# kessel/dune-pnp

Measured on AMD Instinct MI355X. Metric: assembled DOFs/s + BiCGStab iters/s, 3-species PNP on pore.msh-refined, higher is better.
Workload: dtype f64; 1 GPU; config 3: stationary 3-ion PNP, test/pore_pnp/pore.msh refined k=4 x 1 mirrored copies; dofs=2214099, dofs_per_gpu=2214099, mesh_vertices=738033, triangles=1470464, parallelism=mesh partition (RCB) x1, preconditioner=ilu0, colors=4, sell_slots=5176768, blocks=5155025

## Files before the change

### dune-pnp_amd/csrc/assemble.hip

```cpp
#include <cstdlib>

#include <hip/hip_ext.h>

#include "element.h"
#include "kernels.h"

namespace pnp {

namespace {

template <int OP, int KC = 0>
__device__ __forceinline__ void store_block(double *__restrict__ vc, int lane, int s,
                                            const double *Kc) {
  constexpr int NK = OpTraits<OP>::NK;
  static_assert(!KC || OP == OP_PNP, "constant planes: the PNP operator only");
  constexpr int Q0 = KC ? 2 : 0;
#ifdef ASM_STORE_PLAIN
  store_vals<NK, Q0>(vc + size_t(s) * NK * kRows, lane, Kc);
#else
  store_vals_nt<NK, Q0>(vc + size_t(s) * NK * kRows, lane, Kc);
#endif
}

template <int NF>
__device__ __forceinline__ void residual_tail(const AsmArgs &a, int row, unsigned fl,
                                              const double (&R)[NF]) {
  double cv[NF];
#pragma unroll
  for (int f = 0; f < NF; f++) cv[f] = 0.0;
  if (fl & kRowFlagLoad) {
#pragma unroll
    for (int f = 0; f < NF; f++) cv[f] = a.cvec[size_t(row) * NF + f];
  }
#pragma unroll
  for (int f = 0; f < NF; f++) {
    const double rv = R[f] + cv[f];
    a.r[size_t(row) * NF + f] = ((fl >> f) & 1) ? 0.0 : rv;
  }
}

template <int OP, int JAC, int MINW, int FANR>
__global__ __launch_bounds__(256, MINW) void k_assemble(DevLayout L, AsmArgs a) {
  using T = OpTraits<OP>;
  constexpr int NF = T::NF, NK = T::NK;
  const int row = xcd_block(blockIdx.x, gridDim.x, L.xcd_remap) * blockDim.x + threadIdx.x;
  if (row >= L.n_owned) return;
  const int chunk = row / kRows, lane = row % kRows;
  const int off = L.chunk_off[chunk];
  const uint64_t meta = L.rowmeta[row];
  const int len = int(meta & 63);
  const bool closed = (meta >> 6) & 1;
  const unsigned brk = unsigned(meta >> 8);
  const int *__restrict__ cix = L.colidx + off + lane;
  double *__restrict__ vc = a.vals + size_t(off) * NK;

  const double2 pi2 = reinterpret_cast<const double2 *>(L.xy)[row];
  double ui[NF];
#pragma unroll
  for (int f = 0; f < NF; f++) ui[f] = a.x[size_t(row) * NF + f];
  double ai = 0, aq = 0;
  if constexpr (OP == OP_DIFF || OP == OP_DIFF_IE || OP == OP_POISSON) ai = a.aux0[row];
  if constexpr (OP == OP_POISSON) aq = a.aux1[row];
  if constexpr (OP == OP_PB) pb_fifth(ui[0], ai, aq);

  double R[NF], D[NK], P[NK], F[NK];
#pragma unroll
  for (int f = 0; f < NF; f++) R[f] = 0;
#pragma unroll
  for (int v = 0; v < NK; v++) D[v] = P[v] = F[v] = 0;

  auto next_slot = [&](int s) { return (s + 1 < len) ? s + 1 : (closed ? 1 : -1); };
  auto load_nb = [&](int j, double2 &p, double (&u)[NF], double &a0, double &a1) {
// ... 70 lines not shown
      for (int v = 0; v < NK; v++) P[v] = 0;
    }
    pc = pn;
#pragma unroll
    for (int f = 0; f < NF; f++) uc[f] = un[f];
    ac0 = an0;
    ac1 = an1;
    if (tn > 0) {
      pn = pp;
#pragma unroll
      for (int f = 0; f < NF; f++) un[f] = up[f];
      an0 = ap0;
      an1 = ap1;
    }
  }
  if constexpr (JAC) {
    if (closed) {
#pragma unroll
      for (int v = 0; v < NK; v++) F[v] += P[v];
      store_block<OP>(vc, lane, 1, F);
    }
    store_block<OP>(vc, lane, 0, D);
  }
  residual_tail<NF>(a, row, a.rowflag[row], R);
}

#ifndef ASM_SU
#define ASM_SU 4
#endif
template <int OP>
__host__ __device__ constexpr int asm_lds_rec() {
  return 2 + OpTraits<OP>::NF + (OP == OP_DIFF || OP == OP_DIFF_IE || OP == OP_POISSON) +
         (OP == OP_POISSON);
}
template <int OP>
constexpr int asm_kc() {
  return OP == OP_PNP;
}
constexpr int kPipeDw = 11;
template <class P>
__device__ __forceinline__ void lds_dma4(const P *src, uint32_t *dst_wave) {
  __builtin_amdgcn_global_load_lds(
      (const __attribute__((address_space(1))) void *)(src),
      (__attribute__((address_space(3))) void *)(dst_wave), 4, 0, 0);
}
__device__ __forceinline__ int const_ld(const int *p, int i) {
  return ((const __attribute__((address_space(4))) int *)(p))[i];
}
__device__ __forceinline__ int row_block_const(const DevLayout &L, int b, int nwg) {
  return L.blkmap ? const_ld(L.blkmap, xcd_block(b, nwg, 1)) : xcd_block(b, nwg, L.xcd_remap);
}
template <int OP, int JAC, int MINW, int FANR, int SPLIT = FANR, int STAGE = 0, int LDSG = 0,
          int KC = 0, int PIPE = 0>
__global__ __launch_bounds__(256, MINW) void k_assemble_ga(DevLayout L, AsmArgs a) {
  using T = OpTraits<OP>;
  constexpr int NF = T::NF, NK = T::NK, NS = FANR;
  constexpr bool AUX0 = OP == OP_DIFF || OP == OP_DIFF_IE || OP == OP_POISSON;
  constexpr bool AUX1 = OP == OP_POISSON;
  constexpr int RW = asm_lds_rec<OP>();
  static_assert(!PIPE || (JAC && FANR == 9 && !STAGE && !LDSG), "PIPE: the direct Jacobian walk");
  extern __shared__ double srec[];
  __shared__ uint32_t pfb[PIPE ? 4 * kPipeDw * kRows : 1];
  const int ntiles = (L.n_owned + 255) / 256, G = gridDim.x;
  const int wv = PIPE ? __builtin_amdgcn_readfirstlane(int(threadIdx.x) / kRows) : 0;
  const int ln = int(threadIdx.x) % kRows;
  uint32_t *const pw = pfb + (PIPE ? wv * kPipeDw * kRows : 0);
  int tile = blockIdx.x, b0 = -1, b1 = -1, b2 = -1, o0 = 0, o1 = 0, c1 = 0;
  auto tile_blk = [&](int t) { return t < ntiles ? row_block_const(L, t, ntiles) : -1; };
  auto wave_chunk = [&](int b) {
    return (b >= 0 && b * 256 + wv * kRows < L.n_owned) ? b * 4 + wv : -1;
  };
  auto prefetch = [&](int b, int off, int clen) {
    if (wave_chunk(b) < 0) return;
    const int r0 = b * 256 + wv * kRows;
    const int *cix = L.colidx + off + ln;
#pragma unroll
    for (int k = 1; k < NS; k++)
      lds_dma4(cix + (k < clen ? k : 0) * kRows, pw + (k - 1) * kRows);
    const uint32_t *m =
        reinterpret_cast<const uint32_t *>(L.rowmeta + min(r0 + ln, L.n_owned - 1));
    lds_dma4(m, pw + 8 * kRows);
    lds_dma4(m + 1, pw + 9 * kRows);
    lds_dma4(reinterpret_cast<const uint32_t *>(a.rowflag + r0) + (ln >> 2), pw + 10 * kRows);
  };
  if constexpr (PIPE) {
    if (tile >= ntiles) return;
    b0 = tile_blk(tile);
    b1 = tile_blk(tile + G);
    b2 = tile_blk(tile + 2 * G);
    int c0 = 0;
    if (wave_chunk(b0) >= 0) {
      o0 = const_ld(L.chunk_off, wave_chunk(b0));
      c0 = const_ld(L.chunk_len, wave_chunk(b0));
    }
    if (wave_chunk(b1) >= 0) {
      o1 = const_ld(L.chunk_off, wave_chunk(b1));
      c1 = const_ld(L.chunk_len, wave_chunk(b1));
    }
    prefetch(b0, o0, c0);
  }
  int o2 = 0, c2 = 0, b3 = -1;
  const auto advance = [&]() {
    tile += G;
    b0 = b1, o0 = o1;
    b1 = b2, o1 = o2, c1 = c2;
    b2 = b3;
    return b0 >= 0;
  };
  do {
    const int blk = PIPE ? b0 : row_block(L, blockIdx.x, gridDim.x);
    const int row0 = blk * blockDim.x + threadIdx.x;
    const bool live = row0 < L.n_owned;
    if (!PIPE && !LDSG && !live) return;
    const int row = live ? row0 : 0;
    const int chunk = row / kRows, lane = row % kRows;
    int cj[NS];
    uint64_t meta_pf = 0;
    unsigned fl_pf = 0;
    if constexpr (PIPE) {
      asm volatile("s_waitcnt vmcnt(0)" ::: "memory");
#pragma unroll
      for (int k = 1; k < NS; k++) cj[k] = int(pw[(k - 1) * kRows + ln]);
      meta_pf = uint64_t(pw[8 * kRows + ln]) | (uint64_t(pw[9 * kRows + ln]) << 32);
      fl_pf = (pw[10 * kRows + ln] >> (8 * (ln & 3))) & 0xffu;
      asm volatile("s_waitcnt lgkmcnt(0)" ::: "memory");
      prefetch(b1, o1, c1);
      o2 = c2 = 0;
      if (wave_chunk(b2) >= 0) {
        o2 = const_ld(L.chunk_off, wave_chunk(b2));
        c2 = const_ld(L.chunk_len, wave_chunk(b2));
      }
      b3 = tile_blk(tile + 3 * G);
      if (!live) continue;
    }
    const int off = PIPE ? o0 : L.chunk_off[chunk];
    const uint64_t meta = PIPE ? meta_pf : L.rowmeta[row];
    const int len = int(meta & 63);
    const bool closed = (meta >> 6) & 1;
    const unsigned brk = unsigned(meta >> 8);
    double *__restrict__ vc = a.vals + size_t(off) * NK;

    if constexpr (PIPE) {
    } else if constexpr (LDSG) {
      const uint16_t *__restrict__ lix = L.lidx + off + lane;
#pragma unroll
      for (int k = 1; k < NS; k++) {
        const int t = lix[(k < len ? k : 0) * kRows];
        cj[k] = k < len ? t : 0;
      }
    } else {
      const int *__restrict__ cix = L.colidx + off + lane;
#pragma unroll
      for (int k = 1; k < NS; k++) cj[k] = cix[(k < len ? k : 0) * kRows];
    }
    const double2 pi2 = reinterpret_cast<const double2 *>(L.xy)[row];
    double ui[NF];
    load_nf<NF>(a.x, size_t(row), ui);
    double ai = 0, aq = 0;
    if constexpr (AUX0) ai = a.aux0[row];
    if constexpr (AUX1) aq = a.aux1[row];
    if constexpr (OP == OP_PB) pb_fifth(ui[0], ai, aq);
    if constexpr (LDSG) {
      const int u0 = L.uptr[blk], cnt = L.uown[blk];
      constexpr int kSU = ASM_SU;
      int jj[kSU];
#pragma unroll
      for (int u = 0; u < kSU; u++) {
        const int k = int(threadIdx.x) + u * 256;
        jj[u] = k < cnt ? L.ulist[u0 + k] : -1;
      }
      double t[kSU][RW];
#pragma unroll
      for (int u = 0; u < kSU; u++)
        if (jj[u] >= 0) {
          const double2 p = reinterpret_cast<const double2 *>(L.xy)[jj[u]];
          t[u][0] = p.x;
          t[u][1] = p.y;
          double uu[NF];
          load_nf<NF>(a.x, size_t(jj[u]), uu);
#pragma unroll
          for (int f = 0; f < NF; f++) t[u][2 + f] = uu[f];
          if constexpr (AUX0) t[u][2 + NF] = a.aux0[jj[u]];
          if constexpr (AUX1) t[u][3 + NF] = a.aux1[jj[u]];
        }
#pragma unroll
      for (int u = 0; u < kSU; u++)
        if (jj[u] >= 0)
#pragma unroll
          for (int w = 0; w < RW; w++) srec[size_t(int(threadIdx.x) + u * 256) * RW + w] = t[u][w];
      for (int k = int(threadIdx.x) + kSU * 256; k < cnt; k += blockDim.x) {
        const int j = L.ulist[u0 + k];
        const double2 p = reinterpret_cast<const double2 *>(L.xy)[j];
        double u[NF];
        load_nf<NF>(a.x, size_t(j), u);
        double *r = srec + size_t(k) * RW;
        r[0] = p.x;
        r[1] = p.y;
#pragma unroll
        for (int f = 0; f < NF; f++) r[2 + f] = u[f];
        if constexpr (AUX0) r[2 + NF] = a.aux0[j];
        if constexpr (AUX1) r[3 + NF] = a.aux1[j];
      }
      __syncthreads();
      if (!live) return;
    }
    double2 pn[NS];
    double un[NS][NF], a0[NS], a1[NS];
    auto gather = [&](int k) {
      if constexpr (LDSG) {
        const double *r = srec + size_t(cj[k]) * RW;
        pn[k] = make_double2(r[0], r[1]);
#pragma unroll
        for (int f = 0; f < NF; f++) un[k][f] = r[2 + f];
// ... 67 lines not shown
#pragma unroll
              for (int v = 0; v < NK; v++) F[v] = P[v];
            } else {
              put(s, P);
            }
#pragma unroll
            for (int v = 0; v < NK; v++) P[v] = Ct[v];
          }
        } else if constexpr (JAC) {
          put(s, P);
#pragma unroll
          for (int v = 0; v < NK; v++) P[v] = 0;
        }
      }
    }
    if constexpr (JAC) {
      if (closed) {
#pragma unroll
        for (int v = 0; v < NK; v++) F[v] += P[v];
        store_block<OP, KC>(vc, lane, 1, F);
      }
      store_block<OP, KC>(vc, lane, 0, D);
    }
    residual_tail<NF>(a, row, PIPE ? fl_pf : unsigned(a.rowflag[row]), R);
  } while (PIPE && advance());
}

template <int OP>
__global__ __launch_bounds__(256) void k_mass_apply(DevLayout L, double tau, double pi, int cyl,
                                                    const double *__restrict__ xo,
                                                    double *__restrict__ cvec) {
  constexpr int NF = OpTraits<OP>::NF;
  const int row = blockIdx.x * blockDim.x + threadIdx.x;
  if (row >= L.n_owned) return;
  const int chunk = row / kRows, lane = row % kRows;
  const int off = L.chunk_off[chunk];
  const uint64_t meta = L.rowmeta[row];
  const int len = int(meta & 63);
  const bool closed = (meta >> 6) & 1;
  const int *cix = L.colidx + off + lane;
  const double2 pi2 = reinterpret_cast<const double2 *>(L.xy)[row];
  double acc = 0;
  for (int s = 1; s < len; ++s) {
    const int t = (s + 1 < len) ? s + 1 : (closed ? 1 : -1);
    if (t < 0 || ((meta >> (8 + s)) & 1)) continue;
    const int b = cix[s * kRows], c = cix[t * kRows];
    const double2 pb2 = reinterpret_cast<const double2 *>(L.xy)[b];
// ... 74 lines not shown
    static const int resident = [&] {
      int dev = 0, cus = 0, per_cu = 0;
      if (hipGetDevice(&dev) != hipSuccess ||
          hipDeviceGetAttribute(&cus, hipDeviceAttributeMultiprocessorCount, dev) != hipSuccess ||
          hipOccupancyMaxActiveBlocksPerMultiprocessor(&per_cu, kern, 256, 0) != hipSuccess)
        return 0;
      return per_cu * cus;
    }();
    const int ntiles = (L.n_owned + 255) / 256;
    int g = resident >= 8 ? resident / 8 * 8 : 8;
    if (g > ntiles) g = ntiles;
    if (cap > 0 && g > cap) g = cap;
    hipExtLaunchKernelGGL(kern, dim3(g), dim3(256), 0, s, t0, t1, 0, L, a);
    return 1;
  } else {
    return 0;
  }
}

hipError_t launch_assemble(const DevLayout &L, const AsmArgs &a, hipStream_t s, hipEvent_t t0,
                           hipEvent_t t1, int *pipelined) {
  if (pipelined) *pipelined = 0;
  if (L.n_owned == 0) return hipSuccess;
  dim3 grid((L.n_owned + 255) / 256), block(256);
  static const int waves = [] {
    const char *e = getenv("PNP_ASM_WAVES");
    return (e && atoi(e) == 4) ? 4 : 3;
  }();
  static const bool fanr_ok = [] {
    const char *e = getenv("PNP_ASM_FANR");
    return !(e && atoi(e) == 0);
  }();
  static const int ga = [] {
    const char *e = getenv("PNP_ASM_GA");
    return e ? atoi(e) : 4;
  }();
  const int fanr = !fanr_ok ? 0 : (L.max_slots <= 9 ? 9 : (L.max_slots <= 12 ? 12 : 0));
  static const int lds_env = [] {
    const char *e = getenv("PNP_ASM_LDS");
    return e ? (atoi(e) == 1 ? 1 : 0) : -1;
  }();
  static const bool cold_hint = [] {
    const char *e = getenv("PNP_ASM_COLD_HINT");
    return !(e && e[0] == '0');
  }();
  const auto lds_walk = [&](int nk) {
// ... 92 lines not shown
```

### dune-pnp_amd/csrc/ctx.cc

```cpp
#include "ctx.h"

static thread_local std::string g_err;
std::mutex g_groups_m;
std::map<std::string, std::shared_ptr<LocalGroup>> g_groups;

void pnp_ctx::asm_wrote(bool kc, bool full) {
  if (kc) {
    asm_reused++;
  } else {
    asm_full++;
    vals_const_valid = full;
  }
}

pnp_ctx::~pnp_ctx() {
  graphs_clear();
  for (auto &v : ev_pending)
    for (auto &pr : v) {
      hipEventDestroy(pr.first);
      hipEventDestroy(pr.second);
    }
  for (auto e : ev_pool) hipEventDestroy(e);
  if (hS) hipHostFree(hS);
  if (h_send) hipHostFree(h_send);
// ... 1655 lines not shown
  view->bseg = mb->m.bseg.data();
  view->bseg_group = mb->m.bgroup.data();
  return PNP_OK;
}

extern "C" void pnp_mesh_free(pnp_mesh_buf *m) { delete m; }

extern "C" const char *pnp_last_error(const pnp_ctx *ctx) {
  return ctx ? ctx->err.c_str() : g_err.c_str();
}

extern "C" int pnp_rccl_unique_id(void *out128) {
  if (!out128) return PNP_E_ARG;
  ncclUniqueId id;
  if (ncclGetUniqueId(&id) != ncclSuccess) {
    g_err = "ncclGetUniqueId failed";
    return PNP_E_RCCL;
  }
  static_assert(sizeof(ncclUniqueId) == 128, "ncclUniqueId size");
  std::memcpy(out128, &id, 128);
  return PNP_OK;
}

static void params_from(const pnp_params *pp, pnp::Params &P) {
  P.l_b = pp->l_b;
  P.c0 = pp->c0;
  P.tau = pp->tau;
  P.pi = pp->pi;
  P.cylindrical = pp->cylindrical;
  P.surf.resize(pp->n_surfaces);
  for (int i = 0; i < pp->n_surfaces; i++) {
    const pnp_surface &s = pp->surfaces[i];
    pnp::Surface &d = P.surf[i];
    d.cb = s.coulomb_btype;
    d.cflux = s.coulomb_flux;
    d.cpot = s.coulomb_potential;
    d.pb = s.plus_btype;
    d.pflux = s.plus_flux;
    d.pconc = s.plus_concentration;
    d.mb = s.minus_btype;
    d.mflux = s.minus_flux;
    d.mconc = s.minus_concentration;
  }
}

#define CK(expr, what)                                 \
// ... 292 lines not shown
        c->h_posrowU[pos] = rowU(pos);
      }
      c->h_lsx_ptr = lp;
      c->h_lsx_list = ll;
      c->h_usx_ptr = up2;
      c->h_usx_list = ul;
      c->ilu_flow[0].built = c->ilu_flow[1].built = false;
    }
  }
  {
    std::vector<int> ro(L.n_owned + 1, 0), rcol;
    rcol.reserve(size_t(L.nblocks));
    for (int i = 0; i < L.n_owned; i++) {
      const int ch = i / pnp::kRows, ln = i % pnp::kRows, len = pnp::meta_len(L.rowmeta[i]);
      for (int sl = 0; sl < len; sl++)
        rcol.push_back(L.colidx[size_t(L.chunk_off[ch]) + 64 * size_t(sl) + ln]);
      ro[i + 1] = ro[i] + len;
    }
    if ((rc = up(c->d_rowoff, ro, "rowoff")) || (rc = up(c->d_rowcol, rcol, "rowcol"))) {
      g_err = c->err;
      return rc;
    }
  }
  {
    const char *e = getenv("PNP_BLKMAP");
    if (!(e && atoi(e) == 0) && L.n_owned > 0) {
      int nblk = (L.n_owned + 255) / 256;
      std::vector<double> key(nblk);
      for (int b = 0; b < nblk; b++) {
        int r = 256 * b, cc = L.rowcolor[r];
        double lo = L.color_ptr[cc], hi = L.color_ptr[cc + 1];
        key[b] = (r - lo) / std::max(1.0, hi - lo);
      }
      std::vector<int> order(nblk);
      for (int b = 0; b < nblk; b++) order[b] = b;
      std::stable_sort(order.begin(), order.end(), [&](int a, int b) { return key[a] < key[b]; });
      if ((rc = up(c->d_blkmap, order, "blkmap"))) {
        g_err = c->err;
        return rc;
      }
      c->dl.blkmap = c->d_blkmap.p;
    }
  }
  {
    const pnp::Mesh &mg = c->mesh;
    auto ekey = [](int a, int b) {
      if (a > b) std::swap(a, b);
      return (long long)a << 32 | (unsigned)b;
    };
    std::unordered_map<long long, int> opp;
    opp.reserve(size_t(mg.nb) * 2);
    for (int b = 0; b < mg.nb; b++) opp[ekey(mg.bseg[2 * b], mg.bseg[2 * b + 1])] = -1;
    for (int e = 0; e < mg.nt; e++)
      for (int k = 0; k < 3; k++) {
        auto it = opp.find(ekey(mg.tri[3 * e + k], mg.tri[3 * e + (k + 1) % 3]));
        if (it != opp.end() && it->second < 0) it->second = mg.tri[3 * e + (k + 2) % 3];
      }
    std::vector<int4> segs;
    for (int b = 0; b < mg.nb; b++) {
      const int a = mg.bseg[2 * b], cc = mg.bseg[2 * b + 1], lo = L.g2l[std::min(a, cc)];
      if (lo < 0 || lo >= L.n_owned) continue;
      const int o = opp[ekey(a, cc)];
      const int la = L.g2l[a], lc = L.g2l[cc], lop = o >= 0 ? L.g2l[o] : -1;
      if (la < 0 || lc < 0 || lop < 0) {
// ... 86 lines not shown
        const int ch = i / pnp::kRows, ln = i % pnp::kRows;
        for (int sl = 0; sl < L.chunk_len[ch]; sl++) {
          const size_t pos = size_t(L.chunk_off[ch]) + 64 * size_t(sl) + ln;
          lidx[pos] = uint16_t(npos[std::lower_bound(cols.begin(), cols.end(), L.colidx[pos]) - cols.begin()]);
        }
      }
      std::vector<int> reord(cols.size());
      for (size_t k = 0; k < cols.size(); k++) reord[npos[k]] = cols[k];
      ulist.insert(ulist.end(), reord.begin(), reord.end());
      uptr[b + 1] = int(ulist.size());
    }
    if (fits && size_t(umax) * 3 * 8 <= 64 * 1024) {
      if ((rc = up(c->d_uptr, uptr, "uptr")) || (rc = up(c->d_ulist, ulist, "ulist")) ||
          (rc = up(c->d_lidx, lidx, "lidx")) || (rc = up(c->d_uown, uown, "uown"))) {
        g_err = c->err;
        return rc;
      }
      c->dl.uptr = c->d_uptr.p;
      c->dl.ulist = c->d_ulist.p;
      c->dl.lidx = c->d_lidx.p;
      c->dl.umax = umax;
      c->dl.uown = c->d_uown.p;
      c->dl.unmax = unmax;
    }
  }
  c->dl.xy = c->d_xy.p;
  c->dl.color_idx = c->d_color_idx.p;
  c->dl.rowcolor = c->d_rowcolor.p;
  size_t nv3 = 3 * size_t(nloc);
  auto al = [&](auto &buf, size_t n, const char *what) -> int {
    hipError_t e2 = buf.alloc(n);
    if (e2 != hipSuccess) return cp->hipfail(e2, what);
    return PNP_OK;
  };
  if ((rc = al(c->vals, size_t(L.nslots) * 8, "vals")) ||
      (rc = al(c->lu, size_t(L.nslots) * 8, "lu")) ||
      (rc = al(c->lvals, c->d_lsrc.n * 8, "lvals")) || (rc = al(c->uvals, c->d_usrc.n * 8, "uvals")) ||
      (rc = al(c->tsgs, nv3, "sgs scratch")) || (rc = al(c->fluxx, nv3, "flux state")) ||
      (rc = al(c->fluxout, 2 * c->fseg_group.size() + 2, "flux out")) ||
      (rc = al(c->fluxred, 2 * 256, "flux reduce")) || (rc = al(c->x, nv3, "x")) ||
      (rc = al(c->r, nv3, "r")) || (rc = al(c->rs, nv3, "rs")) || (rc = al(c->z, nv3, "z")) || (rc = al(c->rt, nv3, "rt")) ||
      (rc = al(c->p, nv3, "p")) || (rc = al(c->v, nv3, "v")) || (rc = al(c->t, nv3, "t")) ||
      (rc = al(c->y, nv3, "y")) || (rc = al(c->y2, nv3, "y2")) ||
      (rc = al(c->ilu_y32buf, nv3, "ILU(0) intermediate")) || (rc = al(c->b, nv3, "b")) || (rc = al(c->prevu, nv3, "prevu")) ||
      (rc = al(c->ext, 3 * size_t(c->mesh.nv), "ext")) ||
      (rc = al(c->sendbuf, 3 * std::max<size_t>(1, L.send_idx.size()), "sendbuf")) ||
      (rc = al(c->partials,
// ... 1309 lines not shown
  t->assemble_launches = c->t_n[T_ASM];
  t->spmv_launches = c->t_n[T_SPMV];
  t->prec_launches = c->t_n[T_PREC];
  t->blas_launches = c->t_n[T_BLAS];
  t->factor_ms = c->t_ms[T_FACT];
  t->factor_launches = c->t_n[T_FACT];
  return PNP_OK;
}

extern "C" int pnp_timers_reset(pnp_ctx *c) {
  if (!c) return PNP_E_ARG;
  c->timers_flush();
  for (int k = 0; k < T_NCAT; k++) {
    c->t_ms[k] = 0;
    c->t_n[k] = 0;
  }
  return PNP_OK;
}

struct pnp_layout_buf {
  pnp::Fans fans;
  pnp::LocalLayout L;
  std::vector<int> chunk_off32;
};

extern "C" int pnp_setup_boundary(const pnp_mesh *mesh, const pnp_params *params, int32_t nfields,
                                  int32_t field0, uint8_t *mask, double *load) {
  if (!params || nfields < 1 || field0 < 0 || field0 + nfields > 3) return PNP_E_ARG;
  pnp::Mesh m;
  std::string err;
  if (!mesh_from_view(mesh, m, err)) {
    g_err = err;
    return PNP_E_MESH;
  }
  pnp::Params P;
  params_from(params, P);
  for (int s = 0; s < m.nb; s++)
    if (m.bgroup[s] < 0 || m.bgroup[s] >= int(P.surf.size())) return PNP_E_ARG;
  std::vector<uint8_t> mk;
  std::vector<double> ld;
  pnp::dirichlet_mask(m, P, nfields, field0, mk);
  pnp::neumann_load(m, P, nfields, field0, ld);
  for (int v = 0; v < m.nv; v++)
    for (int f = 0; f < nfields; f++) {
      if (mask) mask[size_t(f) * m.nv + v] = mk[size_t(v) * nfields + f];
      if (load) load[size_t(f) * m.nv + v] = ld[size_t(v) * nfields + f];
// ... 17 lines not shown
  pnp::initial_state(m, P, phi_pb, x0);
  return PNP_OK;
}

extern "C" int pnp_layout_build(const pnp_mesh *mesh, int32_t rank, int32_t nranks,
                                pnp_layout_buf **out) {
  if (!out || nranks < 1 || rank < 0 || rank >= nranks) return PNP_E_ARG;
  pnp::Mesh m;
  std::string err;
  if (!mesh_from_view(mesh, m, err)) {
    g_err = err;
    return PNP_E_MESH;
  }
  auto b = std::make_unique<pnp_layout_buf>();
  if (!pnp::build_fans(m, b->fans, err)) {
    g_err = err;
    return PNP_E_MESH;
  }
  std::vector<int> part;
  pnp::rcb_partition(m, nranks, part);
  if (!pnp::build_local_layout(m, b->fans, part, rank, nranks, b->L, err)) {
    g_err = err;
    return PNP_E_MESH;
  }
  *out = b.release();
  return PNP_OK;
}

extern "C" int pnp_layout_view(const pnp_layout_buf *b, pnp_layout *v) {
  if (!b || !v) return PNP_E_ARG;
  const pnp::LocalLayout &L = b->L;
  v->n_owned = L.n_owned;
  v->n_ghost = L.n_ghost;
  v->ncolors = int(L.color_ptr.size()) - 1;
  v->nchunks = L.nchunks;
  v->nnbr = int(L.nbr_ranks.size());
  v->max_slots = b->fans.max_slots;
  v->nslots = L.nslots;
  v->nblocks = L.nblocks;
  v->l2g = L.l2g.data();
  v->color_ptr = L.color_ptr.data();
  v->color_idx = L.color_idx.data();
  v->rowcolor = L.rowcolor.data();
  v->chunk_len = L.chunk_len.data();
  v->chunk_off = L.chunk_off.data();
  v->colidx = L.colidx.data();
  v->rowmeta = L.rowmeta.data();
  v->nbr_ranks = L.nbr_ranks.data();
  v->recv_ptr = L.recv_ptr.data();
  v->send_ptr = L.send_ptr.data();
  v->send_idx = L.send_idx.data();
  v->color_conflicts = L.conflicts;
  return PNP_OK;
}

extern "C" void pnp_layout_free(pnp_layout_buf *b) { delete b; }
```

### dune-pnp_amd/csrc/ctx.h

```cpp
#pragma once

#include <hip/hip_runtime.h>
#include <rccl/rccl.h>
#include <rocsolver/rocsolver.h>

#include <algorithm>
#include <queue>
#include <random>
#include <chrono>
#include <condition_variable>
#include <map>
#include <unordered_map>
#include <mutex>
#include <cmath>
#include <cstdio>
#include <cstdlib>
#include <cstring>
#include <memory>
#include <string>
#include <vector>

#include "../../include/pnp_capi.h"
#include "amg.h"
#include "gmres_small.h"
// ... 150 lines not shown
  DBuf<int> d_lchunk_len, d_lchunk_off, d_lcolidx, d_lsrc, d_uchunk_len, d_uchunk_off, d_ucolidx,
      d_usrc;
  DBuf<double> lvals, uvals, tsgs;
  int ilu_f32 = [] {
    const char *e = std::getenv("PNP_ILU_F32");
    const int v = e ? std::atoi(e) : 2;
    return (v >= 0 && v <= 3) ? v : 2;
  }();
  int ilu_eff() const { return (ilu_f32 >= 2 && nf == 1) ? 1 : ilu_f32; }
  int ilu_fac() const { return ilu_eff() == 3 ? 2 : ilu_eff(); }
  int f32_now() const { return split_of == 2 ? ilu_fac() : 0; }
  DBuf<float> ilu_y32buf;
  float *ilu_y32() const {
    return (split_of == 2 && ilu_eff() == 3 && !ilu_flow_opt) ? ilu_y32buf.p : nullptr;
  }
  int ilu_fused = 1;
  int amg_fallback = 0;
  int ilu_retry = 1;
  int twored_opt = [] {
    const char *ev = std::getenv("PNP_BICG_TWORED");
    return ev ? (std::atoi(ev) != 0 ? 1 : 0) : -1;
  }();
  DBuf<int> d_blkmap;
  DBuf<int> d_rowoff, d_rowcol;
  DBuf<int> d_blk_int, d_blk_bnd;
  int n_blk_int = 0, n_blk_bnd = 0;
  bool split_spmv = false;
  pnp::DevLayout sub_layout(bool interior) const {
    pnp::DevLayout d = dl;
    d.blkmap = interior ? d_blk_int.p : d_blk_bnd.p;
    const int n = interior ? n_blk_int : n_blk_bnd;
    d.blkcount = n > 0 ? n : -1;
    return d;
  }
  hipStream_t cstream = nullptr;
  hipEvent_t ev_ready = nullptr, ev_halo = nullptr;
  DBuf<double> scrub;
  bool fd_built = false, fd_mode = false;
  int fd_opt = 0;
  int fd_ne = 0;
  DBuf<int> fd_etri, fd_cdata;
  DBuf<long long> fd_rptr;
  DBuf<double> fd_jel;
  int csr_pat = -1, csr_nf = 0;
  long long csr_nnz = 0;
  DBuf<int> csr_rowptr, csr_col, csr_src;
// ... 387 lines not shown
```

### dune-pnp_amd/csrc/kernels.h

```cpp
#pragma once

#include <hip/hip_runtime.h>

#include <cstdint>

namespace pnp {

constexpr int kRows = 64;

__device__ __forceinline__ int xcd_block(int b, int nwg, int on = 1) {
  if (!on) return b;
  const int q = nwg / 8, r = nwg % 8, xcd = b % 8;
  return (xcd < r ? xcd * (q + 1) : r * (q + 1) + (xcd - r) * q) + b / 8;
}

typedef double double2_a8 __attribute__((ext_vector_type(2), aligned(8)));
template <int NF>
__device__ __forceinline__ void load_nf(const double *__restrict__ x, size_t j, double (&o)[NF]) {
  const double *b = x + size_t(NF) * j;
  int f = 0;
#pragma unroll
  for (; f + 1 < NF; f += 2) {
    const double2_a8 a = *reinterpret_cast<const double2_a8 *>(b + f);
    o[f] = a.x;
    o[f + 1] = a.y;
  }
  if (f < NF) o[f] = b[f];
}
template <int NF>
__device__ __forceinline__ void store_nf(double *__restrict__ x, size_t j, const double (&v)[NF]) {
  double *b = x + size_t(NF) * j;
  int f = 0;
#pragma unroll
// ... 139 lines not shown
}

struct DevLayout {
  int n_owned = 0, n_local = 0, nchunks = 0, ncolors = 0;
  int max_slots = 0;
  int xcd_remap = 0;
  const int *chunk_len = nullptr;
  const int *chunk_off = nullptr;
  const int *colidx = nullptr;
  const uint64_t *rowmeta = nullptr;
  const double *xy = nullptr;
  const int *color_idx = nullptr;
  const uint8_t *rowcolor = nullptr;
  const int *blkmap = nullptr;
  int blkcount = 0;
  const int *lchunk_len = nullptr, *lchunk_off = nullptr, *lcolidx = nullptr;
  const int *uchunk_len = nullptr, *uchunk_off = nullptr, *ucolidx = nullptr;
  const uint8_t *dmask = nullptr;
  const int *uptr = nullptr, *ulist = nullptr;
  const uint16_t *lidx = nullptr;
  int umax = 0;
  const int *uown = nullptr;
  int unmax = 0;
  const int *lsx_ptr = nullptr, *lsx_list = nullptr, *usx_ptr = nullptr, *usx_list = nullptr;
  const uint8_t *lperm = nullptr, *uperm = nullptr, *lpinv = nullptr, *upinv = nullptr;
  const uint8_t *llen = nullptr, *ulen = nullptr, *ldl = nullptr;
  const uint16_t *lsx_idx = nullptr, *usx_idx = nullptr;
  int sx_max = 0;
};

template <int NF>
__device__ __forceinline__ unsigned row_mask(const DevLayout &L, int row) {
  unsigned dm = 0;
#pragma unroll
  for (int f = 0; f < NF; f++) dm |= unsigned(L.dmask[size_t(row) * NF + f] != 0) << f;
  return dm;
}

constexpr unsigned kRowFlagMask = 7, kRowFlagLoad = 8;

struct AsmArgs {
  int kind;
  int jac;
  double l_b, c0, tau, pi, dt, z;
  int cylindrical;
  const double *x;
  const double *aux0;
  const double *aux1;
  const double *cvec;
  const uint8_t *dmask;
  const uint8_t *rowflag;
  double *r;
// ... 242 lines not shown
```

### dune-pnp_amd/python/pnp_amd/__init__.py

```python
from __future__ import annotations

import ctypes as C
import os
from dataclasses import dataclass

import numpy as np

HERE = os.path.dirname(os.path.abspath(__file__))
PKG_ROOT = os.path.dirname(os.path.dirname(HERE))
REPO_ROOT = os.path.dirname(PKG_ROOT)
LIB_PATH = os.environ.get("PNP_AMD_LIB") or os.path.join(PKG_ROOT, "libpnp_amd.so")
HEADER = os.path.join(REPO_ROOT, "include", "pnp_capi.h")

OK, E_ARG, E_HIP, E_RCCL, E_BREAKDOWN, E_NOT_CONVERGED, E_IO, E_MESH, E_STATE = \
    0, -1, -2, -3, -4, -5, -6, -7, -8
OP_PNP, OP_PNP_IMPLICIT_EULER, OP_PB, OP_DIFF, OP_DIFF_IMPLICIT_EULER, OP_POISSON = range(6)
PREC_NONE, PREC_SSOR, PREC_ILU0, PREC_JACOBI, PREC_AMG, PREC_SSOR_NATURAL = range(6)
METHOD_BICGSTAB, METHOD_CG, METHOD_GMRES, METHOD_FGMRES, METHOD_IDR = 0, 1, 2, 3, 4
(OPT_ILU_F32, OPT_ILU_FUSED_FACTOR, OPT_JAC_FD, OPT_BICG_TWORED, OPT_AMG_FALLBACK,
 OPT_GRAPH, OPT_SEQ_ORDER, OPT_ILU_FLOW, OPT_NAT_FLOW, OPT_ILU_RETRY,
 OPT_GMRES_RESTART, OPT_MATRIX_FREE, OPT_ASM_REUSE_CONST, OPT_IDR_S) = (1, 2, 3, 4, 5, 6, 7, 8,
                                                                        9, 10, 11, 12, 13, 14)
ASM_PIPE_ENV, ASM_PIPE_GRID_ENV = "PNP_ASM_PIPE", "PNP_ASM_PIPE_GRID"
ROW_FLAG_LOAD = 8
# ... 200 lines not shown
class _Timers(C.Structure):
    _fields_ = [("assemble_ms", C.c_double), ("spmv_ms", C.c_double), ("prec_ms", C.c_double),
                ("blas_ms", C.c_double), ("halo_ms", C.c_double), ("allreduce_ms", C.c_double),
                ("assemble_launches", C.c_int64), ("spmv_launches", C.c_int64),
                ("prec_launches", C.c_int64), ("blas_launches", C.c_int64),
                ("factor_ms", C.c_double), ("factor_launches", C.c_int64)]


class _CsrView(C.Structure):
    _fields_ = [("n", C.c_int32), ("nnz", C.c_int64), ("rowptr", C.c_void_p), ("col", C.c_void_p),
                ("val", C.c_void_p)]


class _Layout(C.Structure):
    _fields_ = [("n_owned", C.c_int32), ("n_ghost", C.c_int32), ("ncolors", C.c_int32),
                ("nchunks", C.c_int32), ("nnbr", C.c_int32), ("max_slots", C.c_int32),
                ("nslots", C.c_int64), ("nblocks", C.c_int64),
                ("l2g", C.POINTER(C.c_int32)), ("color_ptr", C.POINTER(C.c_int32)),
                ("color_idx", C.POINTER(C.c_int32)), ("rowcolor", C.POINTER(C.c_uint8)),
                ("chunk_len", C.POINTER(C.c_int32)), ("chunk_off", C.POINTER(C.c_int32)),
                ("colidx", C.POINTER(C.c_int32)), ("rowmeta", C.POINTER(C.c_uint64)),
                ("nbr_ranks", C.POINTER(C.c_int32)), ("recv_ptr", C.POINTER(C.c_int32)),
                ("send_ptr", C.POINTER(C.c_int32)), ("send_idx", C.POINTER(C.c_int32)),
                ("color_conflicts", C.c_int64)]


_LIB = None


def lib():
    global _LIB
    if _LIB is None:
        if not os.path.exists(LIB_PATH):
            raise PnpError(E_IO, f"{LIB_PATH} not built (run __graft_entry__.build() or make -C "
                                 f"dune-pnp_amd)")
        L = C.CDLL(LIB_PATH)
        L.pnp_last_error.restype = C.c_char_p
        L.pnp_last_error.argtypes = [C.c_void_p]
        L.pnp_create.argtypes = [C.POINTER(_Mesh), C.POINTER(_Params), C.c_int32,
                                 C.POINTER(_Comm), C.POINTER(C.c_void_p)]
        L.pnp_create_pk.argtypes = [C.POINTER(_Mesh), C.POINTER(_Params), C.c_int32, C.c_int32,
                                    C.POINTER(_Comm), C.POINTER(C.c_void_p)]
        for name in ("pnp_destroy", "pnp_mesh_free", "pnp_layout_free"):
            getattr(L, name).restype = None
            getattr(L, name).argtypes = [C.c_void_p]
        _LIB = L
    return _LIB
# ... 168 lines not shown
        m = mesh.c()
        _check(lib().pnp_layout_build(C.byref(m), int(rank), int(nranks), C.byref(buf)))
        v = _Layout()
        _check(lib().pnp_layout_view(buf, C.byref(v)))

        def arr(p, n, dt=np.int32):
            return np.ctypeslib.as_array(p, (n,)).astype(dt).copy() if n else np.zeros(0, dt)
        self.n_owned, self.n_ghost = v.n_owned, v.n_ghost
        self.ncolors, self.nchunks, self.max_slots = v.ncolors, v.nchunks, v.max_slots
        self.nslots, self.nblocks = v.nslots, v.nblocks
        self.l2g = arr(v.l2g, v.n_owned + v.n_ghost)
        self.color_ptr = arr(v.color_ptr, v.ncolors + 1)
        self.color_idx = arr(v.color_idx, v.n_owned)
        self.rowcolor = arr(v.rowcolor, v.n_owned + v.n_ghost, np.uint8)
        self.chunk_len = arr(v.chunk_len, v.nchunks)
        self.chunk_off = arr(v.chunk_off, v.nchunks + 1)
        self.colidx = arr(v.colidx, v.nslots)
        self.rowmeta = arr(v.rowmeta, v.n_owned, np.uint64)
        self.nbr_ranks = arr(v.nbr_ranks, v.nnbr)
        self.recv_ptr = arr(v.recv_ptr, v.nnbr + 1)
        self.send_ptr = arr(v.send_ptr, v.nnbr + 1)
        self.send_idx = arr(v.send_idx, int(self.send_ptr[-1]) if v.nnbr else 0)
        self.color_conflicts = int(v.color_conflicts)
        lib().pnp_layout_free(buf)

    def row_len(self, i):
        return int(self.rowmeta[i] & np.uint64(63))

    def row_cols(self, i):
        c, lane = divmod(i, 64)
        L = self.row_len(i)
        return [int(self.colidx[self.chunk_off[c] + s * 64 + lane]) for s in range(L)]


def set_create_option(option, value):
    _check(lib().pnp_set_create_option(option, C.c_int64(value)))


def get_create_option(option):
    v = C.c_int64(0)
    _check(lib().pnp_get_create_option(option, C.byref(v)))
    return v.value


def rccl_unique_id() -> bytes:
    buf = C.create_string_buffer(128)
# ... 342 lines not shown
```

### include/pnp_capi.h

```cpp
#ifndef PNP_CAPI_H
#define PNP_CAPI_H

#include <stdint.h>

#ifdef __cplusplus
extern "C" {
#endif

#define PNP_CAPI_VERSION 1

enum {
  PNP_OK = 0,
  PNP_E_ARG = -1,
  PNP_E_HIP = -2,
  PNP_E_RCCL = -3,
  PNP_E_BREAKDOWN = -4,
  PNP_E_NOT_CONVERGED = -5,
  PNP_E_IO = -6,
  PNP_E_MESH = -7,
  PNP_E_STATE = -8
};

typedef struct pnp_ctx pnp_ctx;

// ... 291 lines not shown

int pnp_setup_boundary(const pnp_mesh *mesh, const pnp_params *params, int32_t nfields,
                       int32_t field0, uint8_t *mask, double *load);
int pnp_setup_initial_state(const pnp_mesh *mesh, const pnp_params *params, const double *phi_pb,
                            double *x0);

typedef struct pnp_layout_buf pnp_layout_buf;
typedef struct {
  int32_t n_owned, n_ghost, ncolors, nchunks, nnbr, max_slots;
  int64_t nslots, nblocks;
  const int32_t *l2g;
  const int32_t *color_ptr;
  const int32_t *color_idx;
  const uint8_t *rowcolor;
  const int32_t *chunk_len;
  const int32_t *chunk_off;
  const int32_t *colidx;
  const uint64_t *rowmeta;
  const int32_t *nbr_ranks;
  const int32_t *recv_ptr;
  const int32_t *send_ptr;
  const int32_t *send_idx;
  int64_t color_conflicts;
} pnp_layout;
int pnp_layout_build(const pnp_mesh *mesh, int32_t rank, int32_t nranks, pnp_layout_buf **out);
int pnp_layout_view(const pnp_layout_buf *b, pnp_layout *view);
void pnp_layout_free(pnp_layout_buf *b);

#ifdef __cplusplus
}
#endif
#endif
```

Measured before the change: 54.16 billion assembled DOFs/s.

## Precompute per-block assembly head records and load row flags early

Builds a host-side per-workgroup head table (block id, chunk offset, chunk length, live rows, unique-list pointers) and uploads it. The non-pipelined assembly kernel then reads these through scalar constant loads instead of chaining blkmap, chunk_off and rowmeta lookups, which is meant to shorten the dependent-load prologue. Row flags are also loaded early, and a wave-uniform ballot skips the load-vector read when no row in the wave needs it. The cost is an extra table, new layout API fields, and a launcher that now rejects layouts without the head table.

```diff
diff --git a/dune-pnp_amd/csrc/assemble.hip b/dune-pnp_amd/csrc/assemble.hip
--- a/dune-pnp_amd/csrc/assemble.hip
+++ b/dune-pnp_amd/csrc/assemble.hip
@@ -39,6 +39,29 @@
   }
 }
 
+template <int NF>
+__device__ __forceinline__ void residual_tail_early(const AsmArgs &a, int row, unsigned fl,
+                                                    const double (&R)[NF]) {
+  double Rt[NF];
+#pragma unroll
+  for (int f = 0; f < NF; f++) {
+    Rt[f] = R[f];
+    asm volatile("" : "+v"(Rt[f]));
+  }
+  if (__builtin_amdgcn_ballot_w64((fl & kRowFlagLoad) != 0) == 0)
+    residual_tail<NF>(a, row, fl & kRowFlagMask, Rt);
+  else
+    residual_tail<NF>(a, row, fl, Rt);
+}
+template <int OP>
+constexpr bool asm_early_flag() {
+#ifdef ASM_TAIL_LATE
+  return false;
+#else
+  return OP != OP_PNP_IE && OP != OP_DIFF_IE;
+#endif
+}
+
 template <int OP, int JAC, int MINW, int FANR>
 __global__ __launch_bounds__(256, MINW) void k_assemble(DevLayout L, AsmArgs a) {
   using T = OpTraits<OP>;
@@ -48,6 +71,9 @@
   const int chunk = row / kRows, lane = row % kRows;
   const int off = L.chunk_off[chunk];
   const uint64_t meta = L.rowmeta[row];
+  constexpr bool EARLY = asm_early_flag<OP>() && !(JAC && MINW == 4);
+  unsigned fl = 0;
+  if constexpr (EARLY) fl = a.rowflag[row];
   const int len = int(meta & 63);
   const bool closed = (meta >> 6) & 1;
   const unsigned brk = unsigned(meta >> 8);
@@ -164,7 +190,10 @@
     }
     store_block<OP>(vc, lane, 0, D);
   }
-  residual_tail<NF>(a, row, a.rowflag[row], R);
+  if constexpr (EARLY)
+    residual_tail_early<NF>(a, row, fl, R);
+  else
+    residual_tail<NF>(a, row, a.rowflag[row], R);
 }
 
 #ifndef ASM_SU
@@ -204,7 +233,7 @@
   extern __shared__ double srec[];
   __shared__ uint32_t pfb[PIPE ? 4 * kPipeDw * kRows : 1];
   const int ntiles = (L.n_owned + 255) / 256, G = gridDim.x;
-  const int wv = PIPE ? __builtin_amdgcn_readfirstlane(int(threadIdx.x) / kRows) : 0;
+  const int wv = __builtin_amdgcn_readfirstlane(int(threadIdx.x) / kRows);
   const int ln = int(threadIdx.x) % kRows;
   uint32_t *const pw = pfb + (PIPE ? wv * kPipeDw * kRows : 0);
   int tile = blockIdx.x, b0 = -1, b1 = -1, b2 = -1, o0 = 0, o1 = 0, c1 = 0;
@@ -249,13 +278,33 @@
     b2 = b3;
     return b0 >= 0;
   };
+  int hblk = 0, hoff = 0, hclen = 0, hlive = 0, hu0 = 0, hcnt = 0;
+  if constexpr (!PIPE) {
+#ifdef ASM_HEAD_OLD
+    hblk = row_block(L, blockIdx.x, gridDim.x);
+    const int r0 = hblk * 256 + int(threadIdx.x);
+    hlive = r0 < L.n_owned ? kRows : 0;
+    hoff = L.chunk_off[(hlive ? r0 : 0) / kRows];
+    if constexpr (LDSG) hu0 = L.uptr[hblk], hcnt = L.uown[hblk];
+#else
+    typedef int int4v __attribute__((ext_vector_type(4)));
+    const int *h = L.asm_head + size_t(blockIdx.x) * kAsmHeadInts;
+    asm volatile("" ::"s"(LDSG ? (const void *)L.lidx : (const void *)L.colidx), "s"(L.rowmeta),
+                 "s"(L.xy), "s"(a.x), "s"(a.rowflag), "s"(a.vals), "s"(a.cylindrical));
+    const int4v rec = ((const __attribute__((address_space(4))) int4v *)(h))[wv];
+    hblk = rec.x;
+    hoff = rec.y;
+    hclen = rec.z & 255;
+    hlive = rec.z >> 8;
+    if constexpr (LDSG) hu0 = const_ld(h, 3), hcnt = const_ld(h, 7);
+#endif
+  }
   do {
-    const int blk = PIPE ? b0 : row_block(L, blockIdx.x, gridDim.x);
-    const int row0 = blk * blockDim.x + threadIdx.x;
-    const bool live = row0 < L.n_owned;
-    if (!PIPE && !LDSG && !live) return;
+    const int blk = PIPE ? b0 : hblk;
+    const int row0 = blk * (PIPE ? int(blockDim.x) : 256) + threadIdx.x;
+    const bool live = PIPE ? row0 < L.n_owned : ln < hlive;
     const int row = live ? row0 : 0;
-    const int chunk = row / kRows, lane = row % kRows;
+    const int lane = PIPE ? row % kRows : ln;
     int cj[NS];
     uint64_t meta_pf = 0;
     unsigned fl_pf = 0;
@@ -275,9 +324,14 @@
       b3 = tile_blk(tile + 3 * G);
       if (!live) continue;
     }
-    const int off = PIPE ? o0 : L.chunk_off[chunk];
+    const int off = PIPE ? o0 : hoff;
     const uint64_t meta = PIPE ? meta_pf : L.rowmeta[row];
     const int len = int(meta & 63);
+#ifdef ASM_HEAD_OLD
+    const int clen = len;
+#else
+    const int clen = hclen;
+#endif
     const bool closed = (meta >> 6) & 1;
     const unsigned brk = unsigned(meta >> 8);
     double *__restrict__ vc = a.vals + size_t(off) * NK;
@@ -287,13 +341,13 @@
       const uint16_t *__restrict__ lix = L.lidx + off + lane;
 #pragma unroll
       for (int k = 1; k < NS; k++) {
-        const int t = lix[(k < len ? k : 0) * kRows];
+        const int t = lix[(k < clen ? k : 0) * kRows];
         cj[k] = k < len ? t : 0;
       }
     } else {
       const int *__restrict__ cix = L.colidx + off + lane;
 #pragma unroll
-      for (int k = 1; k < NS; k++) cj[k] = cix[(k < len ? k : 0) * kRows];
+      for (int k = 1; k < NS; k++) cj[k] = cix[(k < clen ? k : 0) * kRows];
     }
     const double2 pi2 = reinterpret_cast<const double2 *>(L.xy)[row];
     double ui[NF];
@@ -301,9 +355,13 @@
     double ai = 0, aq = 0;
     if constexpr (AUX0) ai = a.aux0[row];
     if constexpr (AUX1) aq = a.aux1[row];
+    constexpr bool EARLY = !PIPE && asm_early_flag<OP>();
+    unsigned fl = fl_pf;
+    if constexpr (EARLY) fl = a.rowflag[row];
+    if (!PIPE && !LDSG && !live) return;
     if constexpr (OP == OP_PB) pb_fifth(ui[0], ai, aq);
     if constexpr (LDSG) {
-      const int u0 = L.uptr[blk], cnt = L.uown[blk];
+      const int u0 = hu0, cnt = hcnt;
       constexpr int kSU = ASM_SU;
       int jj[kSU];
 #pragma unroll
@@ -330,7 +388,7 @@
         if (jj[u] >= 0)
 #pragma unroll
           for (int w = 0; w < RW; w++) srec[size_t(int(threadIdx.x) + u * 256) * RW + w] = t[u][w];
-      for (int k = int(threadIdx.x) + kSU * 256; k < cnt; k += blockDim.x) {
+      for (int k = int(threadIdx.x) + kSU * 256; k < cnt; k += 256) {
         const int j = L.ulist[u0 + k];
         const double2 p = reinterpret_cast<const double2 *>(L.xy)[j];
         double u[NF];
@@ -444,7 +502,10 @@
       }
       store_block<OP, KC>(vc, lane, 0, D);
     }
-    residual_tail<NF>(a, row, PIPE ? fl_pf : unsigned(a.rowflag[row]), R);
+    if constexpr (EARLY)
+      residual_tail_early<NF>(a, row, fl, R);
+    else
+      residual_tail<NF>(a, row, PIPE ? fl : unsigned(a.rowflag[row]), R);
   } while (PIPE && advance());
 }
 
@@ -565,6 +626,7 @@
                            hipEvent_t t1, int *pipelined) {
   if (pipelined) *pipelined = 0;
   if (L.n_owned == 0) return hipSuccess;
+  if (!L.asm_head || L.blkcount != 0) return hipErrorInvalidValue;
   dim3 grid((L.n_owned + 255) / 256), block(256);
   static const int waves = [] {
     const char *e = getenv("PNP_ASM_WAVES");
diff --git a/dune-pnp_amd/csrc/ctx.cc b/dune-pnp_amd/csrc/ctx.cc
--- a/dune-pnp_amd/csrc/ctx.cc
+++ b/dune-pnp_amd/csrc/ctx.cc
@@ -1701,6 +1701,20 @@
   return PNP_OK;
 }
 
+static std::vector<int> spatial_block_order(const pnp::LocalLayout &L) {
+  const int nblk = (L.n_owned + 255) / 256;
+  std::vector<double> key(nblk);
+  for (int b = 0; b < nblk; b++) {
+    int r = 256 * b, cc = L.rowcolor[r];
+    double lo = L.color_ptr[cc], hi = L.color_ptr[cc + 1];
+    key[b] = (r - lo) / std::max(1.0, hi - lo);
+  }
+  std::vector<int> order(nblk);
+  for (int b = 0; b < nblk; b++) order[b] = b;
+  std::stable_sort(order.begin(), order.end(), [&](int a, int b) { return key[a] < key[b]; });
+  return order;
+}
+
 static void params_from(const pnp_params *pp, pnp::Params &P) {
   P.l_b = pp->l_b;
   P.c0 = pp->c0;
@@ -2039,24 +2053,17 @@
       return rc;
     }
   }
+  std::vector<int> h_blkmap, h_uptr, h_uown;
   {
     const char *e = getenv("PNP_BLKMAP");
     if (!(e && atoi(e) == 0) && L.n_owned > 0) {
-      int nblk = (L.n_owned + 255) / 256;
-      std::vector<double> key(nblk);
-      for (int b = 0; b < nblk; b++) {
-        int r = 256 * b, cc = L.rowcolor[r];
-        double lo = L.color_ptr[cc], hi = L.color_ptr[cc + 1];
-        key[b] = (r - lo) / std::max(1.0, hi - lo);
-      }
-      std::vector<int> order(nblk);
-      for (int b = 0; b < nblk; b++) order[b] = b;
-      std::stable_sort(order.begin(), order.end(), [&](int a, int b) { return key[a] < key[b]; });
+      std::vector<int> order = spatial_block_order(L);
       if ((rc = up(c->d_blkmap, order, "blkmap"))) {
         g_err = c->err;
         return rc;
       }
       c->dl.blkmap = c->d_blkmap.p;
+      h_blkmap = std::move(order);
     }
   }
   {
@@ -2189,7 +2196,21 @@
       c->dl.umax = umax;
       c->dl.uown = c->d_uown.p;
       c->dl.unmax = unmax;
-    }
+      h_uptr = std::move(uptr);
+      h_uown = std::move(uown);
+    }
+  }
+  if (L.n_owned > 0) {
+    std::vector<int> head(size_t((L.n_owned + 255) / 256) * pnp::kAsmHeadInts);
+    pnp::asm_head_table(L.n_owned, L.nchunks, L.chunk_off.data(), L.chunk_len.data(),
+                        h_blkmap.empty() ? nullptr : h_blkmap.data(), c->dl.xcd_remap,
+                        h_uptr.empty() ? nullptr : h_uptr.data(),
+                        h_uown.empty() ? nullptr : h_uown.data(), head.data());
+    if ((rc = up(c->d_asm_head, head, "assembly head records"))) {
+      g_err = c->err;
+      return rc;
+    }
+    c->dl.asm_head = c->d_asm_head.p;
   }
   c->dl.xy = c->d_xy.p;
   c->dl.color_idx = c->d_color_idx.p;
@@ -3545,6 +3566,7 @@
   pnp::Fans fans;
   pnp::LocalLayout L;
   std::vector<int> chunk_off32;
+  std::vector<int> blkmap, asm_head;
 };
 
 extern "C" int pnp_setup_boundary(const pnp_mesh *mesh, const pnp_params *params, int32_t nfields,
@@ -3608,6 +3630,12 @@
   if (!pnp::build_local_layout(m, b->fans, part, rank, nranks, b->L, err)) {
     g_err = err;
     return PNP_E_MESH;
+  }
+  if (b->L.n_owned > 0) {
+    b->blkmap = spatial_block_order(b->L);
+    b->asm_head.resize(b->blkmap.size() * pnp::kAsmHeadInts);
+    pnp::asm_head_table(b->L.n_owned, b->L.nchunks, b->L.chunk_off.data(), b->L.chunk_len.data(),
+                        b->blkmap.data(), 0, nullptr, nullptr, b->asm_head.data());
   }
   *out = b.release();
   return PNP_OK;
@@ -3637,6 +3665,9 @@
   v->send_ptr = L.send_ptr.data();
   v->send_idx = L.send_idx.data();
   v->color_conflicts = L.conflicts;
+  v->blkmap = b->blkmap.data();
+  v->asm_head = b->asm_head.data();
+  v->asm_head_ints = pnp::kAsmHeadInts;
   return PNP_OK;
 }
 
diff --git a/dune-pnp_amd/csrc/ctx.h b/dune-pnp_amd/csrc/ctx.h
--- a/dune-pnp_amd/csrc/ctx.h
+++ b/dune-pnp_amd/csrc/ctx.h
@@ -196,6 +196,7 @@
     return ev ? (std::atoi(ev) != 0 ? 1 : 0) : -1;
   }();
   DBuf<int> d_blkmap;
+  DBuf<int> d_asm_head;
   DBuf<int> d_rowoff, d_rowcol;
   DBuf<int> d_blk_int, d_blk_bnd;
   int n_blk_int = 0, n_blk_bnd = 0;
diff --git a/dune-pnp_amd/csrc/kernels.h b/dune-pnp_amd/csrc/kernels.h
--- a/dune-pnp_amd/csrc/kernels.h
+++ b/dune-pnp_amd/csrc/kernels.h
@@ -8,7 +8,7 @@
 
 constexpr int kRows = 64;
 
-__device__ __forceinline__ int xcd_block(int b, int nwg, int on = 1) {
+__host__ __device__ __forceinline__ int xcd_block(int b, int nwg, int on = 1) {
   if (!on) return b;
   const int q = nwg / 8, r = nwg % 8, xcd = b % 8;
   return (xcd < r ? xcd * (q + 1) : r * (q + 1) + (xcd - r) * q) + b / 8;
@@ -194,12 +194,33 @@
   int umax = 0;
   const int *uown = nullptr;
   int unmax = 0;
+  const int *asm_head = nullptr;
   const int *lsx_ptr = nullptr, *lsx_list = nullptr, *usx_ptr = nullptr, *usx_list = nullptr;
   const uint8_t *lperm = nullptr, *uperm = nullptr, *lpinv = nullptr, *upinv = nullptr;
   const uint8_t *llen = nullptr, *ulen = nullptr, *ldl = nullptr;
   const uint16_t *lsx_idx = nullptr, *usx_idx = nullptr;
   int sx_max = 0;
 };
+
+constexpr int kAsmHeadInts = 16;
+inline void asm_head_table(int n_owned, int nchunks, const int *chunk_off, const int *chunk_len,
+                           const int *blkmap, int xcd_remap, const int *uptr, const int *uown,
+                           int *out) {
+  const int nblk = (n_owned + 255) / 256;
+  for (int b = 0; b < nblk; b++) {
+    int *h = out + size_t(b) * kAsmHeadInts;
+    const int blk = blkmap ? blkmap[xcd_block(b, nblk, 1)] : xcd_block(b, nblk, xcd_remap);
+    for (int w = 0; w < 4; w++) {
+      const int ch = 4 * blk + w;
+      const bool live = ch < nchunks && ch * kRows < n_owned;
+      h[4 * w] = blk;
+      h[4 * w + 1] = live ? chunk_off[ch] : 0;
+      const int rows = n_owned - ch * kRows < kRows ? n_owned - ch * kRows : kRows;
+      h[4 * w + 2] = live ? chunk_len[ch] | rows << 8 : 0;
+      h[4 * w + 3] = w == 0 ? (uptr ? uptr[blk] : 0) : (w == 1 ? (uown ? uown[blk] : 0) : 0);
+    }
+  }
+}
 
 template <int NF>
 __device__ __forceinline__ unsigned row_mask(const DevLayout &L, int row) {
diff --git a/dune-pnp_amd/python/pnp_amd/__init__.py b/dune-pnp_amd/python/pnp_amd/__init__.py
--- a/dune-pnp_amd/python/pnp_amd/__init__.py
+++ b/dune-pnp_amd/python/pnp_amd/__init__.py
@@ -246,7 +246,9 @@
                 ("colidx", C.POINTER(C.c_int32)), ("rowmeta", C.POINTER(C.c_uint64)),
                 ("nbr_ranks", C.POINTER(C.c_int32)), ("recv_ptr", C.POINTER(C.c_int32)),
                 ("send_ptr", C.POINTER(C.c_int32)), ("send_idx", C.POINTER(C.c_int32)),
-                ("color_conflicts", C.c_int64)]
+                ("color_conflicts", C.c_int64),
+                ("blkmap", C.POINTER(C.c_int32)), ("asm_head", C.POINTER(C.c_int32)),
+                ("asm_head_ints", C.c_int32)]
 
 
 _LIB = None
@@ -461,6 +463,9 @@
         self.send_ptr = arr(v.send_ptr, v.nnbr + 1)
         self.send_idx = arr(v.send_idx, int(self.send_ptr[-1]) if v.nnbr else 0)
         self.color_conflicts = int(v.color_conflicts)
+        nblk = (v.n_owned + 255) // 256 if v.asm_head_ints else 0
+        self.blkmap = arr(v.blkmap, nblk)
+        self.asm_head = arr(v.asm_head, nblk * v.asm_head_ints).reshape(nblk, max(1, v.asm_head_ints))
         lib().pnp_layout_free(buf)
 
     def row_len(self, i):
diff --git a/include/pnp_capi.h b/include/pnp_capi.h
--- a/include/pnp_capi.h
+++ b/include/pnp_capi.h
@@ -337,6 +337,9 @@
   const int32_t *send_ptr;
   const int32_t *send_idx;
   int64_t color_conflicts;
+  const int32_t *blkmap;
+  const int32_t *asm_head;
+  int32_t asm_head_ints;
 } pnp_layout;
 int pnp_layout_build(const pnp_mesh *mesh, int32_t rank, int32_t nranks, pnp_layout_buf **out);
 int pnp_layout_view(const pnp_layout_buf *b, pnp_layout *view);
```

Measured after the change: 54.00 billion assembled DOFs/s. About the same (-0.3%).
